# NVlabs/CenterPose

Measured on AMD Instinct MI355X. Metric: images/sec at 512x512 DLA-34 (backbone + heat-map decode + post-process + PnP), higher is better.
Workload: dtype f32 via split-f16 (f16x3) MFMA, f32 accumulate

## Files before the change

centerpose_amd/csrc/cp_common.h:

```cpp
#pragma once
#include <hip/hip_runtime.h>
#include <stdint.h>

#include "../../include/centerpose_hip_testing.h"

#if defined(__HIP_DEVICE_COMPILE__) && !defined(__gfx950__)
#error "centerpose_amd device code is written for gfx950 only (raw-buffer range-check semantics, MFMA shapes, LDS-DMA)"
#endif

#define CP_OK 0
#define CP_ERR_INVALID (-1)
#define CP_ERR_LAUNCH (-2)
#define CP_ERR_ALLOC (-3)
#define CP_ERR_STATE (-4)

enum CpAct : int {
    CP_ACT_NONE = 0,
    CP_ACT_RELU = 1,
    CP_ACT_SIGMOID = 2,
    CP_ACT_SIGMOID_FROM = 3,
};

enum CpStore : int {
    CP_STORE_NHWC = 0,
// ... 89 lines not shown
    int fuse_gbase[CP_MAX_HEAD_GROUP];
    int fuse_final;
    int fuse_gsig[CP_MAX_HEAD_GROUP];
    const float* fuse_gbias[CP_MAX_HEAD_GROUP];
    float* fuse_gout[CP_MAX_HEAD_GROUP];
    const unsigned* in_amax[CP_MAX_SRC];
    unsigned* out_amax;
    const float* fuse_w2_inv;
    int dbg;
    const float* offmask;
    const int* row_index;
    int rows_per_image, row_index_stride;
    const float* up_t;
    const float* up_wt;
    int up_ld, up_f;
};

int cp_launch_conv(const ConvParams& p, hipStream_t stream);
int cp_conv_tile_n(int cout);
int cp_conv_variant(const ConvParams& p);
int cp_launch_splitk_epilogue(const ConvParams& p, hipStream_t stream);
void cp_conv_geometry(const ConvParams& p, bool f16x3, int* tiles, int* nk);
const char* cp_conv_variant_name(int v);
#define CP_NUM_CONV_VARIANTS 46
#define CP_VARIANT_HEAD_ROWS 45
#define CP_VARIANT_DECONV_F32 43
#define CP_VARIANT_DECONV16 44
#define CP_VARIANT_STRM16 41
#define CP_VARIANT_LOWC1S 42
#define CP_VARIANT_GRU 26
bool cp_conv16_supported(const ConvParams& p);
int cp_launch_conv16(const ConvParams& p, hipStream_t stream);
int cp_conv16_variant(const ConvParams& p);
bool cp_halo16_supported(const ConvParams& p);
bool cp_halo16_fused_head_supported(const ConvParams& p);
int cp_launch_halo16_fused_head(const ConvParams& p, hipStream_t stream);
bool cp_halo16_gru_supported(const ConvParams& p);
int cp_launch_halo16_gru(const ConvParams& p, hipStream_t stream);
int cp_launch_halo16(const ConvParams& p, int bn, hipStream_t stream);
bool cp_strm16_supported(const ConvParams& p);
int cp_strm16_jobs(const ConvParams& p);
int cp_launch_strm16(const ConvParams& p, hipStream_t stream);
int cp_launch_dcn16(const ConvParams& p, int bn, hipStream_t stream);
bool cp_pw16_supported(const ConvParams& p);
int cp_launch_pw16(const ConvParams& p, hipStream_t stream);
bool cp_dcn16p_supported(const ConvParams& p);
int cp_dcn16p_blocks(const ConvParams& p);
int cp_launch_dcn16p(const ConvParams& p, hipStream_t stream);
bool cp_dcn16p_wide(const ConvParams& p);
#define CP_VARIANT_DCN16S 36
#define CP_VARIANT_M64N64 37
#define CP_VARIANT_DCN16PW 38
bool cp_dcn16s_supported(const ConvParams& p);
int cp_dcn16s_items(const ConvParams& p);
int cp_launch_dcn16s(const ConvParams& p, hipStream_t stream);
int cp_launch_frag16_repack(const void* w16, void* w16f, int CoutPad, int Kpad16, hipStream_t s);
#define CP_VARIANT_DCN16T 39
// ... 217 lines not shown
```

centerpose_amd/csrc/engine_forward.hip:

```cpp
#include "engine_model.h"

using namespace cp_engine;

namespace {

constexpr int kSplitTiles = 128, kSplitTarget = 384;
constexpr long kLeanMinPixels = 32768;

struct Fwd {
    cp_model* m;
    int B;
    hipStream_t s;
    double* gn_stats_out = nullptr;
    const float* gn_in_mr = nullptr;
    const float* gn_in_a = nullptr;
    const float* gn_in_d = nullptr;
    const float* gn_in_gamma = nullptr;
    const float* gn_in_beta = nullptr;
    int role = -1;
    const unsigned* gn_in_amax = nullptr;
    static constexpr int kMaxSlots = CP_AMAX_STRIDE;
    static constexpr size_t kSlotBytes = (size_t)CP_AMAX_SUB * CP_AMAX_STRIDE * sizeof(unsigned);
    Tensor slots_t;
    unsigned* slots = nullptr;
// ... 306 lines not shown
        const float* const some = (const float*)0x1000;
        ConvParams p = conv_params(B, H, W, &some, &C, 1, d.main, 1, 1, CP_ACT_RELU);
        if (p.Cin != d.main.CinP) return false;
        p.offmask = some;
        const unsigned* no_amax = nullptr;
        if (!conv_params_f16(p, d.main, &no_amax, true)) return false;
        p.store = CP_STORE_NHWC;
        p.ldo = d.main.Cout;
        p.up_t = p.up_wt = some;
        p.up_ld = t_c;
        p.up_f = f;
        p.splitk = plan_split(p, true, d.main);
        return p.splitk == 1 && cp_conv16_variant(p) == CP_VARIANT_DCN16T && cp_dcn16t_upadd_supported(p);
    }

    Tensor conv(const ConvW& w, const std::vector<const Tensor*>& srcs, int stride, int pad, int act,
                const Tensor* res = nullptr, const Tensor* offmask = nullptr, int act_from = 0,
                float* out_nchw = nullptr, int out_ld = 0, const UpFuse* up = nullptr) {
        const Tensor& x0 = *srcs[0];
        const int nsrc = (int)srcs.size();
        const float* src[CP_MAX_SRC];
        int src_c[CP_MAX_SRC];
        const unsigned* src_amax[CP_MAX_SRC];
        for (int i = 0; i < nsrc; ++i) {
            src[i] = srcs[i]->ptr();
            src_c[i] = srcs[i]->C;
            src_amax[i] = srcs[i]->amax;
        }
        ConvParams p = conv_params(B, x0.H, x0.W, src, src_c, nsrc, w, stride, pad, act);
        if (p.Cin != w.CinP) {
            chk(fail(CP_ERR_INVALID, "conv: channel mismatch"));
            return Tensor();
        }
// ... 35 lines not shown
            p.ldo = cstore;
            p.coff = 0;
        }
        Tensor partial;
        p.splitk = plan_split(p, use16, w);
        if (p.splitk > 1) {
            partial = make(p.splitk * p.CoutPad, p.Ho, p.Wo);
            p.partial = partial.ptr();
        }
        if (up) {
            p.up_t = up->t->ptr();
            p.up_wt = up->wt;
            p.up_ld = up->t->C;
            p.up_f = up->f;
        }
        auto launch = [&]() -> int {
            int rc = use16 ? cp_launch_conv16(p, s) : cp_launch_conv(p, s);
            if (rc == CP_OK && p.splitk > 1) rc = cp_launch_splitk_epilogue(p, s);
            return rc;
        };
        if (!m->dry)
            timed([&](cp_model::ProfRec& r) {
                r.variant = use16 ? cp_conv16_variant(p) : cp_conv_variant(p);
                r.role = role >= 0 ? role : offmask ? CP_ROLE_DCN : act == CP_ACT_SIGMOID_FROM ? CP_ROLE_DCN_OFFSET
                         : (w.KH == 1 && w.KW == 1) ? CP_ROLE_CONV1X1 : CP_ROLE_CONV;
                const double M = (double)B * p.Ho * p.Wo;
                const int cin_real = w.Cin;
                r.flops = 2.0 * M * w.Cout * (double)(w.KH * w.KW * cin_real);
                r.bytes = 4.0 * ((double)B * x0.H * x0.W * cin_real + M * w.Cout +
                                 (double)w.KH * w.KW * cin_real * w.Cout + (offmask ? M * 27 : 0.0) +
                                 (res ? M * w.Cout : 0.0) + (up ? (double)B * up->t->H * up->t->W * w.Cout : 0.0));
                r.M = (int)M; r.N = w.Cout; r.K = w.KH * w.KW * cin_real; r.kh = w.KH; r.stride = stride;
            }, launch);
        gn_stats_out = nullptr;
        gn_in_mr = nullptr;
        gn_in_a = nullptr;
        gn_in_d = nullptr;
        gn_in_amax = nullptr;
        role = -1;
        return out;
    }
    const ConvW& cw(const std::string& k) { return m->convs.at(k); }

    Tensor maxpool(const Tensor& x) {
        Tensor o = make(x.C, x.H / 2, x.W / 2);
        o.amax = x.amax;
        if (!m->dry) chk(cp_launch_maxpool2(x.ptr(), o.ptr(), B, x.H, x.W, x.C, s));
        return o;
    }

    Tensor basic_block(const std::string& p, const Tensor& x, int stride, const Tensor& residual) {
        Tensor t = conv(cw(p + ".conv1"), {&x}, stride, 1, CP_ACT_RELU);
        Tensor o = conv(cw(p + ".conv2"), {&t}, 1, 1, CP_ACT_RELU, &residual);
        tap(p, o);
        return o;
    }

    Tensor tree1(const std::string& p, const Tensor& x, int cin, int cout, int stride, bool level_root,
                 std::vector<const Tensor*> children, const Tensor* bottom_in = nullptr) {
        Tensor bottom_own;
        const Tensor* bottom = &x;
        if (stride > 1) {
            if (bottom_in) bottom = bottom_in;
            else {
                bottom_own = maxpool(x);
                bottom = &bottom_own;
            }
        }
        Tensor proj;
        const Tensor* residual = bottom;
        if (cin != cout) {
            proj = conv(cw(p + ".project"), {bottom}, 1, 0, CP_ACT_NONE);
            residual = &proj;
        }
        if (level_root) children.insert(children.begin(), bottom);
        Tensor x1 = basic_block(p + ".tree1", x, stride, *residual);
        proj = Tensor();
        Tensor x2 = basic_block(p + ".tree2", x1, 1, x1);
        std::vector<const Tensor*> srcs = {&x2, &x1};
        for (auto* c : children) srcs.push_back(c);
        Tensor o = conv(cw(p + ".root"), srcs, 1, 0, CP_ACT_RELU);
        tap(p + ".root", o);
        return o;
    }
    Tensor tree2(const std::string& p, const Tensor& x, int cin, int cout) {
        Tensor bottom = maxpool(x);
        Tensor x1 = tree1(p + ".tree1", x, cin, cout, 2, false, {}, &bottom);
        return tree1(p + ".tree2", x1, cout, cout, 1, false, {&bottom, &x1});
    }

    Tensor deform(const std::string& p, const Tensor& x, const UpFuse* up = nullptr) {
// ... 503 lines not shown
```

centerpose_amd/csrc/igemm.hip:

```cpp
#include "igemm_common.h"

namespace {

__device__ __forceinline__ float blend(float w1, float v1, float w2, float v2, float w3, float v3, float w4, float v4,
                                       float mk) {
    float s = __fadd_rn(__fadd_rn(__fadd_rn(__fmul_rn(w1, v1), __fmul_rn(w2, v2)), __fmul_rn(w3, v3)),
                        __fmul_rn(w4, v4));
    return __fmul_rn(s, mk);
}

template <int FRAG, int MT, int NT, int WM, int WN, bool DCN, bool ALIGNED, bool MULTISRC>
__global__ __launch_bounds__(NTHREADS, 3) void igemm_kernel(const ConvParams p, const int tiles_m, const int tiles_n) {
    typedef Frag<FRAG> F;
    typedef typename F::acc_t acc_t;
    constexpr int BM = FRAG * MT * WM, BN = FRAG * NT * WN;
    static_assert(WM * WN * 64 == NTHREADS, "4 waves");
    static_assert(!DCN || ALIGNED, "DCN needs aligned channels");
    static_assert(!MULTISRC || (ALIGNED && !DCN), "virtual concat only on the aligned plain-conv path");
    constexpr int LDA = BM + (FRAG == 16 ? 18 : 2);
    constexpr int LDB = BN + (FRAG == 16 ? 0 : 4);
    constexpr int A_SLOTS = BM * BK / 4 / NTHREADS;
    constexpr int B_F4 = BK * BN / 4;
    constexpr int B_SLOTS = (B_F4 + NTHREADS - 1) / NTHREADS;
    constexpr int A_SZ = BK * LDA, B_SZ = BK * LDB;
// ... 421 lines not shown
                      (!p.res || p.res_ld % 4 == 0) && p.splitk <= 32 && slab_bytes * 32 < (size_t)0xf0000000u &&
                      total / 4 < (size_t)0x7fffffff && !(p.dbg & CP_SEL_SPLITK_ELEMENTWISE);
    if (quad) {
        int g = (int)((total / 4 + 255) / 256);
        if (g > 4096) g = 4096;
        hipLaunchKernelGGL(splitk_epilogue4_kernel, dim3(g), dim3(256), 0, stream, p);
        return hipGetLastError() == hipSuccess ? CP_OK : CP_ERR_LAUNCH;
    }
    int g = (int)((total + 255) / 256);
    if (g > 4096) g = 4096;
    hipLaunchKernelGGL(splitk_epilogue_kernel, dim3(g), dim3(256), 0, stream, p);
    return hipGetLastError() == hipSuccess ? CP_OK : CP_ERR_LAUNCH;
}

int cp_launch_conv(const ConvParams& p, hipStream_t stream) {
    if (p.nsrc < 1 || p.nsrc > CP_MAX_SRC || p.Cin % 4 != 0 || p.up_t) return CP_ERR_INVALID;
    for (int s = 0; s < p.nsrc; ++s)
        if (p.src_c[s] % 4 != 0 || (p.nsrc > 1 && p.src_c[s] % BK != 0)) return CP_ERR_INVALID;
    const int bn = cp_conv_tile_n(p.Cout);
    if (p.offmask) {
        if (p.KH != 3 || p.KW != 3 || p.stride != 1 || p.pad != 1 || p.nsrc != 1 || p.Cin % BK != 0 ||
            p.H != p.Ho || p.W != p.Wo)
            return CP_ERR_INVALID;
        if (bn == 128) return launch<32, 2, 2, 2, 2, true>(p, stream);
        if (bn == 64) return launch<32, 2, 1, 2, 2, true>(p, stream);
        return CP_ERR_INVALID;
    }
    switch (bn) {
        case 16: return launch<16, 4, 1, 4, 1, false>(p, stream);
        case 32: return launch<32, 2, 1, 4, 1, false>(p, stream);
        case 64: return launch<32, 2, 1, 2, 2, false>(p, stream);
// ... 4 lines not shown
```

centerpose_amd/csrc/igemm16.hip:

```cpp
#include "igemm16_common.h"

namespace {

template <int MT, int NT, int WM, int WN, bool MULTISRC, bool FUSE = false, bool GNIN = false, bool GRU = false, bool ROWS = false>
__global__ __launch_bounds__(WM * WN * 64, 2) void igemm16p_kernel(const ConvParams p, const int tiles_m, const int tiles_n) {
    static_assert(!FUSE || (MT == 2 && NT == 2 && WM == 2 && WN == 2 && !MULTISRC), "fused head: 128x128 tiles");
    static_assert(!GRU || (MT == 1 && NT == 3 && WM == 4 && WN == 1 && !MULTISRC && !FUSE), "GRU: 128x96 tiles");
    static_assert(!ROWS || FUSE, "pixel lists: fused heads only");
    typedef Frag<32> F;
    typedef F::acc_t acc_t;
    constexpr int BM = 32 * MT * WM, BN = 32 * NT * WN;
    constexpr int NTH = WM * WN * 64;
    constexpr int RPP = NTH / 8;
    constexpr int A_SLOTS = BM * BK16 / 4 / NTH;
    constexpr int B_CHUNKS = BN * BK16 * 2 / 16;
    constexpr int B_SLOTS = (B_CHUNKS + NTH - 1) / NTH;
    constexpr bool B_PART = B_CHUNKS % NTH != 0;
    constexpr int A_SZ = BM * LDH, B_SZ = BN * LDH;
    constexpr int BUF = 2 * A_SZ + 2 * B_SZ;
    constexpr int NM = 3 * MT * NT;
    constexpr int NR = 2 * MT + 2 * NT;
    __shared__ __attribute__((aligned(16))) _Float16 lds[2 * BUF];

    const int tid = threadIdx.x;
// ... 539 lines not shown
    return (p.dbg & CP_SEL_DCN16S_ALWAYS) || cp_dcn16s_items(p) >= 4096;
}

static bool dcn16t_wanted(const ConvParams& p) {
    if ((p.dbg & CP_SEL_DCN16T_NEVER) || !dcn16p_wanted(p) || !cp_dcn16t_supported(p)) return false;
    if (p.dbg & CP_SEL_DCN16T_ALWAYS) return true;
    if (p.dbg & CP_SEL_DCN16S_ALWAYS) return false;
    return !cp_dcn16p_wide(p) && cp_dcn16p_blocks(p) >= 1024;
}

static bool strm16_wanted(const ConvParams& p) {
    if ((p.dbg & CP_SEL_STRM16_NEVER) || (p.dbg & CP_SEL_HALO_NEVER) || !cp_strm16_supported(p)) return false;
    return (p.dbg & CP_SEL_STRM16_ALWAYS) || cp_strm16_jobs(p) >= 1024;
}

static bool halo16_wanted(const ConvParams& p, int bn) {
    if ((p.dbg & CP_SEL_HALO_NEVER) || p.gn_in_a || !cp_halo16_supported(p)) return false;
    return bn == 32 || (p.w16f_hi && p.w16f_lo && !(p.dbg & CP_SEL_HALO_LDS_WEIGHTS)) || (p.dbg & CP_SEL_HALO_ALWAYS);
}

static bool pw16_wanted(const ConvParams& p) { return !(p.dbg & CP_SEL_PW16_NEVER) && cp_pw16_supported(p); }

bool cp_conv16_supported(const ConvParams& p) {
    if (!p.w16_hi || !p.w16_lo || p.Cin % BK16 != 0 || p.KH * p.KW > 32) return false;
    for (int s = 0; s < p.nsrc; ++s)
        if (p.src_c[s] % BK16 != 0) return false;
    const int bn = conv16_tile_n(p);
    if (bn < 32) return false;
    if (p.gn_in_mr) return false;
    if (p.gn_in_a || p.gn_in_d) {
        if (!p.gn_in_a || !p.gn_in_d || bn != 32 || p.KH != 1 || p.KW != 1 || p.pad != 0 || p.stride != 1 || p.nsrc != 1 ||
            p.offmask || (p.Ho * p.Wo) % 128 != 0)
            return false;
    }
    if (p.offmask && bn < 64) return false;
    for (int s = 0; s < p.nsrc; ++s)
        if ((size_t)p.B * p.H * p.W * p.src_c[s] * 4 >= (size_t)0xf0000000u) return false;
    if ((size_t)p.CoutPad * p.Kpad16 * 2 >= ((size_t)1 << 32)) return false;
    return true;
}

int cp_launch_conv16(const ConvParams& p, hipStream_t stream) {
    if (!cp_conv16_supported(p)) return CP_ERR_INVALID;
    if (p.up_t && !(p.offmask && dcn16t_wanted(p) && cp_dcn16t_upadd_supported(p))) return CP_ERR_INVALID;
    const int bn = conv16_tile_n(p);
    const bool cat = p.nsrc > 1;
    if (p.gn_in_a) {
        const int M = p.B * p.Ho * p.Wo;
        const int tiles_m = (M + 127) / 128, tiles_n = p.CoutPad / 32;
        hipLaunchKernelGGL((igemm16p_kernel<1, 1, 4, 1, false, false, true>),
                           dim3(tiles_m * tiles_n, p.splitk > 1 ? p.splitk : 1), dim3(NT16), 0, stream, p, tiles_m, tiles_n);
        return hipGetLastError() == hipSuccess ? CP_OK : CP_ERR_LAUNCH;
    }
    if (p.offmask) {
        if (p.KH != 3 || p.KW != 3 || p.stride != 1 || p.pad != 1 || p.nsrc != 1 || p.H != p.Ho || p.W != p.Wo)
            return CP_ERR_INVALID;
        if (dcn16t_wanted(p)) return cp_launch_dcn16t(p, stream);
        if (dcn16s_wanted(p)) return cp_launch_dcn16s(p, stream);
        if (dcn16p_wanted(p)) return cp_launch_dcn16p(p, stream);
// ... 112 lines not shown
```

centerpose_amd/csrc/ops.hip:

```cpp
#include "engine_model.h"

using namespace cp_engine;

namespace {

struct Carve {
    char* base;
    size_t off = 0;
    template <class T>
    T* take(size_t bytes) {
        T* p = base ? (T*)(base + off) : nullptr;
        off += align_up(bytes, 256);
        return p;
    }
};

constexpr size_t kSlotBytes = (size_t)CP_AMAX_SUB * CP_AMAX_STRIDE * sizeof(unsigned);

struct Pack16 {
    void *hi, *lo;
    float *wfwd, *winv, *sc16;
    unsigned* slot;
    void *fhi, *flo;
};
// ... 335 lines not shown
    d.wf = r.wf;
    d.hi = r.hi;
    d.lo = r.lo;
    d.scale = scale;
    d.scale16 = r.sc16;
    d.shift = shift;
    d.Cin = Cin;
    d.Cout = Cout;
    rc = cp_launch_deconv(deconv_launch(d, f16x3, x, f16x3 ? r.slot : nullptr, B, H, W, out, nullptr, act == CP_ACT_RELU), s);
    return rc == CP_OK ? CP_OK : fail(rc, "deconv launch failed (shape too large for 32-bit offsets?)");
}

int cp_conv2d_nhwc(cp_stream_t stream, const float* x, const float* w, const float* scale, const float* shift,
                   const float* residual, float* out, int B, int H, int W, int Cin, int Cout, int KH, int KW,
                   int stride, int pad, int act, void* workspace, size_t workspace_bytes) {
    if (!x || !w || !out || !workspace) return fail(CP_ERR_INVALID, "null argument");
    if (Cin % 4) return fail(CP_ERR_INVALID, "Cin must be a multiple of 4");
    Carve c{(char*)workspace};
    const Conv2dWs r = conv2d_carve(c, Cin, Cout, KH, KW);
    if (workspace_bytes < c.off) return fail(CP_ERR_INVALID, "workspace too small");
    hipStream_t s = (hipStream_t)stream;
    const int bn = cp_conv_tile_n(Cout);
    ConvW cw = conv_w_f32(r.wp, scale, shift, Cin, Cout, KH, KW);
    if ((scale || shift) && cw.CoutPad != Cout) return fail(CP_ERR_INVALID, "scale/shift need Cout % tile_n == 0");
    if (hipMemsetAsync(r.wp, 0, (size_t)cw.Kpad * cw.CoutPad * sizeof(float), s) != hipSuccess) return CP_ERR_LAUNCH;
    int rc = cp_launch_pack_weight(w, r.wp, Cout, Cin, KH * KW, Cin, cw.CoutPad, 0, s);
    if (rc != CP_OK) return rc;
    ConvParams p = conv_params(B, H, W, &x, &Cin, 1, cw, stride, pad, act);
    p.res = residual;
    p.res_ld = Cout;
    p.out = out;
    p.store = CP_STORE_NHWC;
    p.ldo = Cout;
    if (g_default_precision == CP_PREC_F16X3 && Cin % 32 == 0 && KH * KW <= 32 && bn >= 32) {
        rc = pack_f16x3(r.f16, w, scale, KH * KW, cw, x, (size_t)B * H * W * Cin, nullptr, 0, s);
        if (rc != CP_OK) return rc;
        const unsigned* slot = r.f16.slot;
        if (conv_params_f16(p, cw, &slot, true)) return cp_launch_conv16(p, s);
    }
    return cp_launch_conv(p, s);
}

size_t cp_conv2d_backward_workspace_bytes(int B, int H, int W, int Cin, int Cout, int KH, int KW, int stride, int pad,
                                          int need_grad_x) {
    if (const char* e = conv_bwd_shape_error(B, H, W, Cin, Cout, KH, KW, stride, pad)) {
        fail(CP_ERR_INVALID, e);
        return 0;
    }
    return cp_conv_backward_ws_bytes(B, H, W, Cin, Cout, KH, KW, stride, pad, need_grad_x);
}

int cp_conv2d_backward_nhwc(cp_stream_t stream, const float* x, const float* w, const float* y_or_null, const float* grad_out,
                            float* grad_x_or_null, float* grad_w, float* grad_bias_or_null, int B, int H, int W, int Cin,
                            int Cout, int KH, int KW, int stride, int pad, void* workspace, size_t workspace_bytes) {
// ... 133 lines not shown
```

centerpose_amd/hip.py:

```python
import contextlib
import ctypes
import enum
import os
from collections import OrderedDict
from collections.abc import Mapping

import torch

_HERE = os.path.dirname(os.path.abspath(__file__))
LIB_PATH = os.environ.get("CENTERPOSE_HIP_LIB") or os.path.join(_HERE, "libcenterpose_hip.so")

_lib = None
ABI_VERSION = 7

c_void_p = ctypes.c_void_p
c_int = ctypes.c_int
c_size_t = ctypes.c_size_t
c_char_p = ctypes.c_char_p


class TrackParams(ctypes.Structure):
    _fields_ = [(n, ctypes.c_double) for n in ("new_thresh", "pre_thresh", "R", "conf_lo", "conf_hi")] + \
               [(n, ctypes.c_int) for n in ("max_age", "kalman", "scale_pool", "use_pnp", "hps_uncertainty", "show_axes",
                                            "cat_rule", "render_hm_mode", "render_hmhp_mode", "pre_hm", "pre_hm_hp", "K",
# ... 76 lines not shown
         ctypes.POINTER(c_void_p))
    _sig(L.cp_model_set_param, c_int, c_void_p, c_char_p, c_void_p, ctypes.c_int64)
    _sig(L.cp_model_finalize, c_int, c_void_p)
    _sig(L.cp_model_destroy, None, c_void_p)
    _sig(L.cp_model_workspace_bytes, c_size_t, c_void_p, c_int, c_int, c_int)
    _sig(L.cp_model_forward, c_int, c_void_p, c_void_p, c_int, c_int, c_int, c_void_p, c_void_p, c_void_p, c_void_p,
         ctypes.POINTER(c_void_p), c_int, c_void_p, c_size_t)
    _sig(L.cp_model_forward_tap, c_int, c_void_p, c_void_p, c_int, c_int, c_int, c_void_p, c_void_p, c_void_p,
         c_void_p, ctypes.POINTER(c_void_p), c_int, c_void_p, c_size_t, c_char_p, c_void_p, ctypes.POINTER(c_int))
    _sig(L.cp_conv2d_workspace_bytes, c_size_t, c_int, c_int, c_int, c_int)
    _sig(L.cp_conv_transpose2d_workspace_bytes, c_size_t, c_int, c_int)
    _sig(L.cp_conv_transpose2d_nhwc, c_int, c_void_p, c_void_p, c_void_p, c_void_p, c_void_p, c_void_p,
         c_int, c_int, c_int, c_int, c_int, c_int, c_void_p, c_size_t)
    _sig(L.cp_conv2d_nhwc, c_int, c_void_p, c_void_p, c_void_p, c_void_p, c_void_p, c_void_p, c_void_p,
         *([c_int] * 10), c_void_p, c_size_t)
    _sig(L.cp_conv2d_backward_workspace_bytes, c_size_t, *([c_int] * 10))
    _sig(L.cp_conv2d_backward_nhwc, c_int, *([c_void_p] * 8), *([c_int] * 9), c_void_p, c_size_t)
    _sig(L.cp_batchnorm_workspace_bytes, c_size_t, *([c_int] * 4))
    _sig(L.cp_batchnorm_forward_nhwc, c_int, *([c_void_p] * 10), *([c_int] * 5), ctypes.c_float, ctypes.c_float, c_int, c_void_p,
         c_size_t)
    _sig(L.cp_batchnorm_backward_nhwc, c_int, *([c_void_p] * 11), *([c_int] * 5), c_void_p, c_size_t)
    _sig(L.cp_decode_workspace_bytes, c_size_t, c_int, c_int)
    _sig(L.cp_decode, c_int, c_void_p, c_int, c_int, c_int, *([c_void_p] * 11), c_int, c_int, c_int, ctypes.c_float,
         c_int, c_int, c_void_p, c_void_p, c_size_t)
    _sig(L.cp_decode_tiled_workspace_bytes, c_size_t, c_int, c_int, c_int, c_int)
    _sig(L.cp_decode_tiled, c_int, c_void_p, c_int, c_int, c_int, *([c_void_p] * 11), c_int, c_int, c_int, ctypes.c_float,
         c_int, c_int, c_void_p, c_void_p, c_size_t)
    _sig(L.cp_model_detect_workspace_bytes, c_size_t, c_void_p, c_int, c_int, c_int, c_int)
    _sig(L.cp_model_detect, c_int, c_void_p, c_void_p, c_int, c_int, c_int, c_void_p, c_void_p, c_void_p, c_void_p,
         ctypes.POINTER(c_void_p), c_int, c_int, c_int, ctypes.c_float, c_int, c_void_p, c_void_p, c_size_t, c_int)
# ... 69 lines not shown
            "cp_model_forward", "cp_model_forward_tap", "cp_conv2d_workspace_bytes", "cp_conv2d_nhwc",
            "cp_decode_workspace_bytes", "cp_decode", "cp_pnp_workspace_bytes", "cp_pnp_solve", "cp_model_profile", "cp_model_profile_read",
            "cp_kernel_variant_name", "cp_set_default_precision", "cp_model_set_precision", "cp_model_detect_workspace_bytes", "cp_model_detect", "cp_set_debug", "cp_preprocess", "cp_preprocess_batch", "cp_postprocess_workspace_bytes", "cp_postprocess", "cp_render_gaussians",
            "cp_model_profile_roles", "cp_role_name", "cp_pnp_from_post_workspace_bytes", "cp_pnp_from_post", "cp_resize_u8",
            "cp_abi_version", "cp_num_kernel_variants", "cp_num_roles", "cp_track_state_bytes", "cp_track_workspace_bytes",
            "cp_track_reset", "cp_track_step", "cp_track_status", "cp_linear_assignment", "cp_decode_tiled_workspace_bytes",
            "cp_decode_tiled", "cp_box_iou", "cp_box_eval", "cp_conv_transpose2d_workspace_bytes",
            "cp_conv_transpose2d_nhwc", "cp_dcnv2_backward_workspace_bytes", "cp_dcnv2_backward",
            "cp_pose_loss_workspace_bytes", "cp_pose_loss_forward", "cp_pose_loss_backward",
            "cp_pose_targets_workspace_bytes", "cp_pose_targets", "cp_model_lean_supported",
            "cp_model_detect_lean_workspace_bytes", "cp_model_detect_lean", "cp_model_dense_heads",
            "cp_model_heads_at_workspace_bytes", "cp_model_heads_at", "cp_decode_peaks_workspace_bytes", "cp_decode_peaks",
            "cp_decode_gathered", "cp_pose_heads_chunk_images", "cp_pose_heads_forward_workspace_bytes",
            "cp_pose_heads_forward", "cp_pose_heads_backward_workspace_bytes", "cp_pose_heads_backward",
            "cp_model_features", "cp_conv2d_backward_workspace_bytes", "cp_conv2d_backward_nhwc",
            "cp_batchnorm_workspace_bytes", "cp_batchnorm_forward_nhwc", "cp_batchnorm_backward_nhwc"]


def _check(rc, what):
    if rc != 0:
        msg = lib().cp_last_error().decode() if _lib is not None else ""
        raise RuntimeError("centerpose_hip: %s failed with code %d (%s)" % (what, rc, msg))


class KernelSel(enum.IntFlag):
    HEADS_SLABS = 0x00000001
    HEADS_WG_PER_HEAD = 0x00000002
    PW16_FRAG_A = 0x00000004
    SPLITK_ELEMENTWISE = 0x00000008
    TILE128_SMALL = 0x00000010
    NO_HEAD_FUSION = 0x00000020
# ... 165 lines not shown
    if need_feat_grad and grad_feat is None:
        grad_feat = torch.empty_like(feat, memory_format=torch.channels_last)
    if need_feat_grad and not (grad_feat.is_cuda and grad_feat.dtype == torch.float32 and grad_feat.shape == feat.shape and
                               grad_feat.is_contiguous(memory_format=torch.channels_last)):
        raise RuntimeError("pose_heads_backward: grad_feat must be a float32 channels_last tensor of feat's shape")
    nbytes = L.cp_pose_heads_backward_workspace_bytes(B, H, W, Cin, hid, n, cls_arr)
    if nbytes == 0:
        raise RuntimeError("pose_heads_backward: shape refused by the library (%s)" % L.cp_last_error().decode())
    ws = torch.empty(nbytes, dtype=torch.uint8, device=feat.device)
    rc = L.cp_pose_heads_backward(_stream(), _ptr(feat), n, *tables, cls_arr, goptr, *gtab,
                                  _ptr(grad_feat) if need_feat_grad else c_void_p(0), B, H, W, Cin, hid, _ptr(ws), nbytes)
    _check(rc, "cp_pose_heads_backward")
    return (grad_feat if need_feat_grad else None), grads


def conv2d_nhwc(x, w, scale=None, shift=None, residual=None, stride=1, pad=0, act=0):
    L = lib()
    x, w = _dev(x), _dev(w)
    B, H, W, Cin = x.shape
    Cout, _, KH, KW = w.shape
    Ho = (H + 2 * pad - KH) // stride + 1
    Wo = (W + 2 * pad - KW) // stride + 1
    out = torch.empty(B, Ho, Wo, Cout, device=x.device, dtype=torch.float32)
    nbytes = L.cp_conv2d_workspace_bytes(Cin, Cout, KH, KW)
    ws = torch.empty(nbytes, dtype=torch.uint8, device=x.device)
    scale = _dev(scale) if scale is not None else None
    shift = _dev(shift) if shift is not None else None
    residual = _dev(residual) if residual is not None else None
    rc = L.cp_conv2d_nhwc(_stream(), _ptr(x), _ptr(w), _ptr(scale), _ptr(shift), _ptr(residual), _ptr(out),
                          B, H, W, Cin, Cout, KH, KW, stride, pad, act, _ptr(ws), nbytes)
    _check(rc, "cp_conv2d_nhwc")
    return out


def conv2d_backward(x, w, grad_out, stride=1, pad=0, y=None, need_x_grad=True, need_bias_grad=True):
    L = lib()
    x, w, grad_out = _dev(x), _dev(w), _dev(grad_out)
    y = _dev(y) if y is not None else None
    if x.dim() != 4 or w.dim() != 4 or w.shape[1] != x.shape[3]:
        raise RuntimeError("conv2d_backward: x must be [B,H,W,Cin] and w [Cout,Cin,KH,KW], got %s and %s"
                           % (tuple(x.shape), tuple(w.shape)))
    B, H, W, Cin = x.shape
    Cout, _, KH, KW = w.shape
# ... 1082 lines not shown
```

include/centerpose_hip.h:

```cpp
#ifndef CENTERPOSE_HIP_H
#define CENTERPOSE_HIP_H

#include <stddef.h>
#include <stdint.h>

#ifdef __cplusplus
extern "C" {
#endif

typedef void* cp_stream_t;
typedef struct cp_model cp_model;

#define CP_OK 0
#define CP_ERR_INVALID (-1)
#define CP_ERR_LAUNCH (-2)
#define CP_ERR_ALLOC (-3)
#define CP_ERR_STATE (-4)

#define CP_ABI_VERSION 7
const char* cp_version(void);
int cp_abi_version(void);
const char* cp_last_error(void);

size_t cp_dcnv2_workspace_bytes(int B, int C, int H, int W, int Co);
// ... 77 lines not shown
#define CP_ROLE_HEAD 4
#define CP_ROLE_HEAD_FINAL 5
#define CP_ROLE_GRU 6
#define CP_ROLE_LOWC 7
#define CP_ROLE_DECODE 8
#define CP_ROLE_DECONV 9
#define CP_NUM_ROLES 10
int cp_num_roles(void);
int cp_model_profile_roles(cp_model* m, double* out, int num_roles);
const char* cp_role_name(int role);

size_t cp_conv2d_workspace_bytes(int Cin, int Cout, int KH, int KW);
int cp_conv2d_nhwc(cp_stream_t stream, const float* x, const float* w, const float* scale, const float* shift,
                   const float* residual, float* out, int B, int H, int W, int Cin, int Cout, int KH, int KW,
                   int stride, int pad, int act, void* workspace, size_t workspace_bytes);

size_t cp_conv2d_backward_workspace_bytes(int B, int H, int W, int Cin, int Cout, int KH, int KW, int stride, int pad,
                                          int need_grad_x);
int cp_conv2d_backward_nhwc(cp_stream_t stream, const float* x, const float* w, const float* y_or_null,
                            const float* grad_out, float* grad_x_or_null, float* grad_w, float* grad_bias_or_null, int B,
                            int H, int W, int Cin, int Cout, int KH, int KW, int stride, int pad, void* workspace,
                            size_t workspace_bytes);

size_t cp_batchnorm_workspace_bytes(int B, int H, int W, int C);
int cp_batchnorm_forward_nhwc(cp_stream_t stream, const float* x, const float* gamma_or_null, const float* beta_or_null,
                              const float* residual_or_null, float* running_mean_or_null, float* running_var_or_null,
                              float* y, float* save_mean, float* save_invstd, int B, int H, int W, int C, int training,
                              float momentum, float eps, int act, void* workspace, size_t workspace_bytes);
int cp_batchnorm_backward_nhwc(cp_stream_t stream, const float* x, const float* y_or_null, const float* grad_out,
                               const float* gamma_or_null, const float* save_mean, const float* save_invstd,
// ... 168 lines not shown
```

Measured before the change: 4539.

## Fuse 2x2 maxpool into streamed stride-2 3x3 conv kernel for tree entry

Adds a dedicated streamed stride-2 3x3 conv kernel (Cin 32 to Cout 64, split-f16 MFMA) that also writes the 2x2 max-pooled input as a side output. It is used at the DLA tree entry, where the stride-2 conv1 and the maxpool for the bottom path read the same input. This removes a separate maxpool launch and a second read of the large input tensor. The new kernel keeps weights in LDS, streams input rows through per-wave LDS buffers, and adds a selection heuristic and a new public API entry point. In exchange there is more special-case code, and it applies only to one narrow layer shape.

```diff
diff --git a/centerpose_amd/csrc/cp_common.h b/centerpose_amd/csrc/cp_common.h
--- a/centerpose_amd/csrc/cp_common.h
+++ b/centerpose_amd/csrc/cp_common.h
@@ -127,6 +127,7 @@
     const float* up_t;
     const float* up_wt;
     int up_ld, up_f;
+    float* pool_out;
 };
 
 int cp_launch_conv(const ConvParams& p, hipStream_t stream);
@@ -154,6 +155,10 @@
 bool cp_strm16_supported(const ConvParams& p);
 int cp_strm16_jobs(const ConvParams& p);
 int cp_launch_strm16(const ConvParams& p, hipStream_t stream);
+bool cp_igemm16s2_supported(const ConvParams& p);
+int cp_igemm16s2_jobs(const ConvParams& p);
+int cp_launch_igemm16s2(const ConvParams& p, hipStream_t stream);
+bool cp_conv16_pool_fusable(const ConvParams& p);
 int cp_launch_dcn16(const ConvParams& p, int bn, hipStream_t stream);
 bool cp_pw16_supported(const ConvParams& p);
 int cp_launch_pw16(const ConvParams& p, hipStream_t stream);
diff --git a/centerpose_amd/csrc/engine_forward.hip b/centerpose_amd/csrc/engine_forward.hip
--- a/centerpose_amd/csrc/engine_forward.hip
+++ b/centerpose_amd/csrc/engine_forward.hip
@@ -344,9 +344,22 @@
         return p.splitk == 1 && cp_conv16_variant(p) == CP_VARIANT_DCN16T && cp_dcn16t_upadd_supported(p);
     }
 
+    bool pool_fusable(const ConvW& w, int C, int H, int W) {
+        if (m->precision != CP_PREC_F16X3) return false;
+        const float* const some = (const float*)0x1000;
+        ConvParams p = conv_params(B, H, W, &some, &C, 1, w, 2, 1, CP_ACT_RELU);
+        if (p.Cin != w.CinP) return false;
+        const unsigned* no_amax = nullptr;
+        if (!conv_params_f16(p, w, &no_amax, true)) return false;
+        p.store = CP_STORE_NHWC;
+        p.ldo = w.Cout;
+        p.splitk = plan_split(p, true, w);
+        return p.splitk == 1 && cp_conv16_pool_fusable(p);
+    }
+
     Tensor conv(const ConvW& w, const std::vector<const Tensor*>& srcs, int stride, int pad, int act,
                 const Tensor* res = nullptr, const Tensor* offmask = nullptr, int act_from = 0,
-                float* out_nchw = nullptr, int out_ld = 0, const UpFuse* up = nullptr) {
+                float* out_nchw = nullptr, int out_ld = 0, const UpFuse* up = nullptr, const Tensor* pool = nullptr) {
         const Tensor& x0 = *srcs[0];
         const int nsrc = (int)srcs.size();
         const float* src[CP_MAX_SRC];
@@ -412,6 +425,7 @@
             p.up_ld = up->t->C;
             p.up_f = up->f;
         }
+        if (pool) p.pool_out = pool->ptr();
         auto launch = [&]() -> int {
             int rc = use16 ? cp_launch_conv16(p, s) : cp_launch_conv(p, s);
             if (rc == CP_OK && p.splitk > 1) rc = cp_launch_splitk_epilogue(p, s);
@@ -427,7 +441,8 @@
                 r.flops = 2.0 * M * w.Cout * (double)(w.KH * w.KW * cin_real);
                 r.bytes = 4.0 * ((double)B * x0.H * x0.W * cin_real + M * w.Cout +
                                  (double)w.KH * w.KW * cin_real * w.Cout + (offmask ? M * 27 : 0.0) +
-                                 (res ? M * w.Cout : 0.0) + (up ? (double)B * up->t->H * up->t->W * w.Cout : 0.0));
+                                 (res ? M * w.Cout : 0.0) + (up ? (double)B * up->t->H * up->t->W * w.Cout : 0.0) +
+                                 (pool ? M * cin_real : 0.0));
                 r.M = (int)M; r.N = w.Cout; r.K = w.KH * w.KW * cin_real; r.kh = w.KH; r.stride = stride;
             }, launch);
         gn_stats_out = nullptr;
@@ -449,6 +464,9 @@
 
     Tensor basic_block(const std::string& p, const Tensor& x, int stride, const Tensor& residual) {
         Tensor t = conv(cw(p + ".conv1"), {&x}, stride, 1, CP_ACT_RELU);
+        return basic_block_tail(p, t, residual);
+    }
+    Tensor basic_block_tail(const std::string& p, const Tensor& t, const Tensor& residual) {
         Tensor o = conv(cw(p + ".conv2"), {&t}, 1, 1, CP_ACT_RELU, &residual);
         tap(p, o);
         return o;
@@ -456,11 +474,16 @@
 
     Tensor tree1(const std::string& p, const Tensor& x, int cin, int cout, int stride, bool level_root,
                  std::vector<const Tensor*> children, const Tensor* bottom_in = nullptr) {
-        Tensor bottom_own;
+        Tensor bottom_own, entry;
         const Tensor* bottom = &x;
         if (stride > 1) {
             if (bottom_in) bottom = bottom_in;
-            else {
+            else if (stride == 2 && pool_fusable(cw(p + ".tree1.conv1"), x.C, x.H, x.W)) {
+                bottom_own = make(x.C, x.H / 2, x.W / 2);
+                bottom_own.amax = x.amax;
+                entry = conv(cw(p + ".tree1.conv1"), {&x}, 2, 1, CP_ACT_RELU, nullptr, nullptr, 0, nullptr, 0, nullptr, &bottom_own);
+                bottom = &bottom_own;
+            } else {
                 bottom_own = maxpool(x);
                 bottom = &bottom_own;
             }
@@ -472,7 +495,8 @@
             residual = &proj;
         }
         if (level_root) children.insert(children.begin(), bottom);
-        Tensor x1 = basic_block(p + ".tree1", x, stride, *residual);
+        Tensor x1 = entry.valid() ? basic_block_tail(p + ".tree1", entry, *residual) : basic_block(p + ".tree1", x, stride, *residual);
+        entry = Tensor();
         proj = Tensor();
         Tensor x2 = basic_block(p + ".tree2", x1, 1, x1);
         std::vector<const Tensor*> srcs = {&x2, &x1};
diff --git a/centerpose_amd/csrc/igemm.hip b/centerpose_amd/csrc/igemm.hip
--- a/centerpose_amd/csrc/igemm.hip
+++ b/centerpose_amd/csrc/igemm.hip
@@ -459,7 +459,7 @@
 }
 
 int cp_launch_conv(const ConvParams& p, hipStream_t stream) {
-    if (p.nsrc < 1 || p.nsrc > CP_MAX_SRC || p.Cin % 4 != 0 || p.up_t) return CP_ERR_INVALID;
+    if (p.nsrc < 1 || p.nsrc > CP_MAX_SRC || p.Cin % 4 != 0 || p.up_t || p.pool_out) return CP_ERR_INVALID;
     for (int s = 0; s < p.nsrc; ++s)
         if (p.src_c[s] % 4 != 0 || (p.nsrc > 1 && p.src_c[s] % BK != 0)) return CP_ERR_INVALID;
     const int bn = cp_conv_tile_n(p.Cout);
diff --git a/centerpose_amd/csrc/igemm16.hip b/centerpose_amd/csrc/igemm16.hip
--- a/centerpose_amd/csrc/igemm16.hip
+++ b/centerpose_amd/csrc/igemm16.hip
@@ -577,6 +577,11 @@
     return (p.dbg & CP_SEL_STRM16_ALWAYS) || cp_strm16_jobs(p) >= 1024;
 }
 
+bool cp_conv16_pool_fusable(const ConvParams& p) {
+    if ((p.dbg & CP_SEL_HALO_NEVER) || !cp_conv16_supported(p) || !cp_igemm16s2_supported(p)) return false;
+    return (p.dbg & CP_SEL_HALO_ALWAYS) || cp_igemm16s2_jobs(p) >= 1024;
+}
+
 static bool halo16_wanted(const ConvParams& p, int bn) {
     if ((p.dbg & CP_SEL_HALO_NEVER) || p.gn_in_a || !cp_halo16_supported(p)) return false;
     return bn == 32 || (p.w16f_hi && p.w16f_lo && !(p.dbg & CP_SEL_HALO_LDS_WEIGHTS)) || (p.dbg & CP_SEL_HALO_ALWAYS);
@@ -606,6 +611,8 @@
 int cp_launch_conv16(const ConvParams& p, hipStream_t stream) {
     if (!cp_conv16_supported(p)) return CP_ERR_INVALID;
     if (p.up_t && !(p.offmask && dcn16t_wanted(p) && cp_dcn16t_upadd_supported(p))) return CP_ERR_INVALID;
+    if (cp_conv16_pool_fusable(p)) return cp_launch_igemm16s2(p, stream);
+    if (p.pool_out) return CP_ERR_INVALID;
     const int bn = conv16_tile_n(p);
     const bool cat = p.nsrc > 1;
     if (p.gn_in_a) {
diff --git a/centerpose_amd/csrc/igemm16s2.hip b/centerpose_amd/csrc/igemm16s2.hip
--- /dev/null
+++ b/centerpose_amd/csrc/igemm16s2.hip
@@ -0,0 +1,258 @@
+#include "igemm16_common.h"
+
+namespace {
+
+constexpr int S2_W = 32;
+constexpr int S2_PITCH = 80;
+constexpr int S2_ODD = 34 * S2_PITCH;
+constexpr int S2_EVEN = 32 * S2_PITCH;
+constexpr int S2_ROWB = S2_ODD + S2_EVEN;
+constexpr int S2_G = 18;
+constexpr int S2_NF = 2;
+constexpr int S2_WB = 2 * S2_NF * S2_G * 1024;
+constexpr int S2_TAB = 128 * 4;
+constexpr int S2_WAVES = 8;
+constexpr int S2_LDS = S2_WB + S2_TAB + S2_WAVES * 2 * S2_ROWB;
+constexpr int S2_XP = 272;
+constexpr int S2_NLD = 9;
+static_assert(S2_LDS + 64 <= 160 * 1024, "one workgroup per CU");
+static_assert(32 * S2_XP <= 2 * S2_ROWB, "the output exchange lives in the wave's row buffer");
+
+__global__ __launch_bounds__(64 * S2_WAVES, 1) void igemm16s2_kernel(const ConvParams p, const int rows, const int strips,
+                                                                     const int bands, const int njobs) {
+    float* const pool_out = p.pool_out;
+    typedef Frag<32> F;
+    typedef F::acc_t acc_t;
+    extern __shared__ __attribute__((aligned(16))) unsigned char smem[];
+    const int tid = threadIdx.x, lane = tid & 63;
+    const int wid = __builtin_amdgcn_readfirstlane(tid >> 6);
+    float afwd, ainv;
+    conv_in_scale(p, &afwd, &ainv);
+    afwd = __uint_as_float(__builtin_amdgcn_readfirstlane(__float_as_uint(afwd)));
+    ainv = __uint_as_float(__builtin_amdgcn_readfirstlane(__float_as_uint(ainv)));
+    {
+        const u32x4* gh = reinterpret_cast<const u32x4*>(p.w16f_hi);
+        const u32x4* gl = reinterpret_cast<const u32x4*>(p.w16f_lo);
+        u32x4* ws = reinterpret_cast<u32x4*>(smem);
+        for (int i = tid; i < S2_NF * S2_G * 64; i += 64 * S2_WAVES) {
+            ws[i] = gh[i];
+            ws[S2_NF * S2_G * 64 + i] = gl[i];
+        }
+        float* tab = reinterpret_cast<float*>(smem + S2_WB);
+        if (tid < 64) {
+            tab[tid] = (p.scale ? p.scale[tid] : 1.f) * ainv;
+            tab[64 + tid] = p.shift ? p.shift[tid] : 0.f;
+        }
+    }
+    __syncthreads();
+    unsigned char* row_hi = smem + S2_WB + S2_TAB + wid * (2 * S2_ROWB);
+    unsigned char* row_lo = row_hi + S2_ROWB;
+    const unsigned char* w_hi = smem + lane * 16;
+    const unsigned char* w_lo = w_hi + S2_NF * S2_G * 1024;
+    const unsigned char* tab_b = smem + S2_WB;
+    const int px = lane & 31, kg = lane >> 5;
+    const int pr = lane >> 3, cq = lane & 7;
+    const unsigned img_b = (unsigned)p.H * (unsigned)p.W * 128u;
+    const float relu_floor = p.act == CP_ACT_RELU ? 0.f : -__builtin_inff();
+    const unsigned pool_b = pool_out ? (unsigned)p.Ho * (unsigned)p.Wo * 128u : 0u;
+    const int st_even = S2_ODD + pr * S2_PITCH + cq * 8, st_odd = (pr + 1) * S2_PITCH + cq * 8;
+    const int st_first = (pr == 0 ? 0 : 33) * S2_PITCH + cq * 8;
+    float amax = 0.f;
+
+    for (int job = wid * (int)gridDim.x + (int)blockIdx.x; job < njobs; job += (int)gridDim.x * S2_WAVES) {
+        int t = job;
+        const int sx = t % strips;
+        t /= strips;
+        const int band = t % bands, b = t / bands;
+        const int x0 = sx * S2_W, y0 = band * rows, y1 = min(y0 + rows, p.Ho);
+        const int j_first = 2 * y0 - 1, j_last = 2 * y1 - 1;
+        const __amdgpu_buffer_rsrc_t r_in = make_rsrc(p.src[0] + (size_t)b * p.H * p.W * 32, img_b);
+        const __amdgpu_buffer_rsrc_t r_out = make_rsrc(p.out + (size_t)b * p.Ho * p.Wo * p.ldo + p.coff, (unsigned)p.Ho * (unsigned)p.Wo * (unsigned)p.ldo * 4u);
+        const __amdgpu_buffer_rsrc_t r_pool = make_rsrc(pool_out ? pool_out + (size_t)b * p.Ho * p.Wo * 32 : p.out, pool_b);
+        unsigned cvo[S2_NLD];
+#pragma unroll
+        for (int k = 0; k < 4; ++k) {
+            const int c = 2 * (x0 + pr + 8 * k);
+            cvo[k] = c < p.W ? (unsigned)(c * 128 + cq * 16) : 0xffffffffu;
+            cvo[4 + k] = c < p.W ? (unsigned)((c + 1) * 128 + cq * 16) : 0xffffffffu;
+        }
+        cvo[8] = (pr == 0 && x0 > 0) ? (unsigned)((2 * x0 - 1) * 128 + cq * 16) : 0xffffffffu;
+        float4 pf[2][S2_NLD];
+        auto request = [&](int j, float4 (&v)[S2_NLD]) {
+            const bool row_ok = (j >= j_first) & (j <= j_last) & ((unsigned)j < (unsigned)p.H);
+            const int so = row_ok ? j * p.W * 128 : 0;
+#pragma unroll
+            for (int k = 0; k < S2_NLD; ++k) {
+                const u32x4 x = __builtin_amdgcn_raw_buffer_load_b128(r_in, (int)(row_ok ? cvo[k] : 0xffffffffu), so, 0);
+                v[k] = make_float4(__uint_as_float(x.x), __uint_as_float(x.y), __uint_as_float(x.z), __uint_as_float(x.w));
+            }
+        };
+        request(j_first - 1, pf[0]);
+        __builtin_amdgcn_sched_barrier(0);
+        request(j_first, pf[1]);
+        __builtin_amdgcn_sched_barrier(0);
+        acc_t acc0[S2_NF], acc1[S2_NF];
+#pragma unroll
+        for (int nf = 0; nf < S2_NF; ++nf)
+#pragma unroll
+            for (int r = 0; r < F::NACC; ++r) acc0[nf][r] = acc1[nf][r] = 0.f;
+        float4 hm[4];
+
+        auto stage = [&](const float4 (&buf)[S2_NLD]) {
+#pragma unroll
+            for (int k = 0; k < S2_NLD; ++k) {
+                const float4 v = buf[k];
+                const Split2 s0 = split2(v.x * afwd, v.y * afwd), s1 = split2(v.z * afwd, v.w * afwd);
+                const int o = k < 4 ? st_even + k * 8 * S2_PITCH : k < 8 ? st_odd + (k - 4) * 8 * S2_PITCH : st_first;
+                *reinterpret_cast<u32x2*>(row_hi + o) = u32x2{s0.hi, s1.hi};
+                *reinterpret_cast<u32x2*>(row_lo + o) = u32x2{s0.lo, s1.lo};
+            }
+        };
+        auto max4 = [](const float4& a, const float4& c) {
+            return make_float4(fmaxf(a.x, c.x), fmaxf(a.y, c.y), fmaxf(a.z, c.z), fmaxf(a.w, c.w));
+        };
+
+        for (int m = y0 - 1; m < y1; ++m) {
+            stage(pf[0]);
+#pragma unroll
+            for (int k = 0; k < 4; ++k) hm[k] = max4(pf[0][k], pf[0][4 + k]);
+            request(2 * m + 2, pf[0]);
+            __builtin_amdgcn_wave_barrier();
+#pragma unroll
+            for (int kw = 0; kw < 3; ++kw)
+#pragma unroll
+                for (int cg = 0; cg < 2; ++cg) {
+                    const int ao = (kw == 1 ? S2_ODD + px * S2_PITCH : (px + (kw >> 1)) * S2_PITCH) + cg * 32 + kg * 16;
+                    const h8 ah = *reinterpret_cast<const h8*>(row_hi + ao), al = *reinterpret_cast<const h8*>(row_lo + ao);
+                    h8 wh[S2_NF], wl[S2_NF];
+#pragma unroll
+                    for (int nf = 0; nf < S2_NF; ++nf) {
+                        const int g = nf * S2_G + (3 + kw) * 2 + cg;
+                        wh[nf] = *reinterpret_cast<const h8*>(w_hi + g * 1024);
+                        wl[nf] = *reinterpret_cast<const h8*>(w_lo + g * 1024);
+                    }
+#pragma unroll
+                    for (int nf = 0; nf < S2_NF; ++nf) acc0[nf] = __builtin_amdgcn_mfma_f32_32x32x16_f16(wh[nf], al, acc0[nf], 0, 0, 0);
+#pragma unroll
+                    for (int nf = 0; nf < S2_NF; ++nf) acc0[nf] = __builtin_amdgcn_mfma_f32_32x32x16_f16(wl[nf], ah, acc0[nf], 0, 0, 0);
+#pragma unroll
+                    for (int nf = 0; nf < S2_NF; ++nf) acc0[nf] = __builtin_amdgcn_mfma_f32_32x32x16_f16(wh[nf], ah, acc0[nf], 0, 0, 0);
+                }
+            __builtin_amdgcn_wave_barrier();
+            stage(pf[1]);
+            const unsigned okm = ~(unsigned)((m - y0) >> 31);
+            {
+                const unsigned prow = (unsigned)(m * p.Wo) * 128u, row_no = ~okm & 0x80000000u;
+#pragma unroll
+                for (int k = 0; k < 4; ++k) {
+                    const float4 v = max4(hm[k], max4(pf[1][k], pf[1][4 + k]));
+                    const int xo = x0 + pr + 8 * k;
+                    const unsigned col_no = xo < p.Wo ? 0u : 0x80000000u;
+                    const u32x4 pk = {__float_as_uint(v.x), __float_as_uint(v.y), __float_as_uint(v.z), __float_as_uint(v.w)};
+                    __builtin_amdgcn_raw_buffer_store_b128(pk, r_pool, (int)((prow + (unsigned)(xo * 128 + cq * 16)) | row_no | col_no), 0, 0);
+                }
+            }
+            request(2 * m + 3, pf[1]);
+            __builtin_amdgcn_wave_barrier();
+#pragma unroll
+            for (int kw = 0; kw < 3; ++kw)
+#pragma unroll
+                for (int cg = 0; cg < 2; ++cg) {
+                    const int ao = (kw == 1 ? S2_ODD + px * S2_PITCH : (px + (kw >> 1)) * S2_PITCH) + cg * 32 + kg * 16;
+                    const h8 ah = *reinterpret_cast<const h8*>(row_hi + ao), al = *reinterpret_cast<const h8*>(row_lo + ao);
+                    h8 wh[2][S2_NF], wl[2][S2_NF];
+#pragma unroll
+                    for (int nf = 0; nf < S2_NF; ++nf) {
+                        const int g2 = nf * S2_G + (6 + kw) * 2 + cg, g0 = nf * S2_G + kw * 2 + cg;
+                        wh[0][nf] = *reinterpret_cast<const h8*>(w_hi + g2 * 1024);
+                        wl[0][nf] = *reinterpret_cast<const h8*>(w_lo + g2 * 1024);
+                        wh[1][nf] = *reinterpret_cast<const h8*>(w_hi + g0 * 1024);
+                        wl[1][nf] = *reinterpret_cast<const h8*>(w_lo + g0 * 1024);
+                    }
+#pragma unroll
+                    for (int nf = 0; nf < S2_NF; ++nf) {
+                        acc0[nf] = __builtin_amdgcn_mfma_f32_32x32x16_f16(wh[0][nf], al, acc0[nf], 0, 0, 0);
+                        acc1[nf] = __builtin_amdgcn_mfma_f32_32x32x16_f16(wh[1][nf], al, acc1[nf], 0, 0, 0);
+                    }
+#pragma unroll
+                    for (int nf = 0; nf < S2_NF; ++nf) {
+                        acc0[nf] = __builtin_amdgcn_mfma_f32_32x32x16_f16(wl[0][nf], ah, acc0[nf], 0, 0, 0);
+                        acc1[nf] = __builtin_amdgcn_mfma_f32_32x32x16_f16(wl[1][nf], ah, acc1[nf], 0, 0, 0);
+                    }
+#pragma unroll
+                    for (int nf = 0; nf < S2_NF; ++nf) {
+                        acc0[nf] = __builtin_amdgcn_mfma_f32_32x32x16_f16(wh[0][nf], ah, acc0[nf], 0, 0, 0);
+                        acc1[nf] = __builtin_amdgcn_mfma_f32_32x32x16_f16(wh[1][nf], ah, acc1[nf], 0, 0, 0);
+                    }
+                }
+            __builtin_amdgcn_wave_barrier();
+            const float okf = __uint_as_float(okm & __float_as_uint(x0 + px < p.Wo ? 1.f : 0.f));
+#pragma unroll
+            for (int nf = 0; nf < S2_NF; ++nf)
+#pragma unroll
+                for (int g4 = 0; g4 < 4; ++g4) {
+                    const int n0 = 32 * nf + 8 * g4 + 4 * kg;
+                    const float4 sc = *reinterpret_cast<const float4*>(tab_b + n0 * 4), sh = *reinterpret_cast<const float4*>(tab_b + 256 + n0 * 4);
+                    float v[4] = {acc0[nf][4 * g4] * sc.x + sh.x, acc0[nf][4 * g4 + 1] * sc.y + sh.y,
+                                  acc0[nf][4 * g4 + 2] * sc.z + sh.z, acc0[nf][4 * g4 + 3] * sc.w + sh.w};
+#pragma unroll
+                    for (int e = 0; e < 4; ++e) {
+                        v[e] = fmaxf(v[e], relu_floor);
+                        amax = fmaxf(amax, fabsf(v[e]) * okf);
+                    }
+                    *reinterpret_cast<float4*>(row_hi + px * S2_XP + n0 * 4) = make_float4(v[0], v[1], v[2], v[3]);
+                }
+            __builtin_amdgcn_wave_barrier();
+            const unsigned row_out = (unsigned)(m * p.Wo * p.ldo) * 4u, row_no = ~okm & 0x80000000u;
+#pragma unroll
+            for (int i = 0; i < 8; ++i) {
+                const int pxo = (lane >> 4) + 4 * i;
+                const u32x4 pk = *reinterpret_cast<const u32x4*>(row_hi + pxo * S2_XP + (lane & 15) * 16);
+                const unsigned col_no = x0 + pxo < p.Wo ? 0u : 0x80000000u;
+                __builtin_amdgcn_raw_buffer_store_b128(pk, r_out, (int)((row_out + (unsigned)(((x0 + pxo) * p.ldo + (lane & 15) * 4) * 4)) | row_no | col_no), 0, 0);
+            }
+            __builtin_amdgcn_wave_barrier();
+#pragma unroll
+            for (int nf = 0; nf < S2_NF; ++nf) {
+                acc0[nf] = acc1[nf];
+#pragma unroll
+                for (int r = 0; r < F::NACC; ++r) acc1[nf][r] = 0.f;
+            }
+        }
+    }
+    if (p.out_amax) cp_amax_commit(p.out_amax, amax);
+}
+
+}
+
+bool cp_igemm16s2_supported(const ConvParams& p) {
+    return p.w16f_hi && p.w16f_lo && p.KH == 3 && p.KW == 3 && p.stride == 2 && p.pad == 1 && p.nsrc == 1 && p.Cin == 32 &&
+           p.src_c[0] == 32 && p.CoutPad == 64 && p.Cout == 64 && !p.offmask && !p.res && !p.gn_stats && !p.gn_in_a && !p.gn_in_mr &&
+           !p.gru_x3 && !p.fuse_w2_hi && !p.up_t && p.splitk <= 1 && p.tile_m != 64 && p.H % 2 == 0 && p.W % 2 == 0 && p.H >= 2 && p.W >= 2 &&
+           p.Ho == p.H / 2 && p.Wo == p.W / 2 && p.store == CP_STORE_NHWC && p.ldo % 4 == 0 && p.coff % 4 == 0 && p.coff + 64 <= p.ldo &&
+           p.Kpad16 == 288 && (p.act == CP_ACT_NONE || p.act == CP_ACT_RELU) &&
+           (size_t)p.H * p.W * 128 < (size_t)0x70000000u && (size_t)p.Ho * p.Wo * p.ldo * 4 < (size_t)0x70000000u;
+}
+
+int cp_igemm16s2_jobs(const ConvParams& p) { return p.B * ((p.Wo + S2_W - 1) / S2_W) * ((p.Ho + 15) / 16); }
+
+int cp_launch_igemm16s2(const ConvParams& p, hipStream_t stream) {
+    if (!cp_igemm16s2_supported(p)) return CP_ERR_INVALID;
+    static int cus_of[16] = {0};
+    int dev = 0;
+    if (hipGetDevice(&dev) != hipSuccess || dev < 0 || dev >= 16) return CP_ERR_LAUNCH;
+    if (!cus_of[dev]) {
+        hipDeviceProp_t prop;
+        if (hipFuncSetAttribute(reinterpret_cast<const void*>(&igemm16s2_kernel), hipFuncAttributeMaxDynamicSharedMemorySize, S2_LDS) != hipSuccess)
+            return CP_ERR_LAUNCH;
+        cus_of[dev] = (hipGetDeviceProperties(&prop, dev) == hipSuccess && prop.multiProcessorCount > 0) ? prop.multiProcessorCount : 256;
+    }
+    const int cus = cus_of[dev];
+    const int strips = (p.Wo + S2_W - 1) / S2_W;
+    const int rows = cp_igemm16s2_jobs(p) >= cus * S2_WAVES * 3 / 4 ? 16 : 8;
+    const int bands = (p.Ho + rows - 1) / rows;
+    const int njobs = p.B * strips * bands;
+    const int blocks = njobs < cus ? njobs : cus;
+    hipLaunchKernelGGL(igemm16s2_kernel, dim3(blocks), dim3(64 * S2_WAVES), S2_LDS, stream, p, rows, strips, bands, njobs);
+    return hipGetLastError() == hipSuccess ? CP_OK : CP_ERR_LAUNCH;
+}
diff --git a/centerpose_amd/csrc/ops.hip b/centerpose_amd/csrc/ops.hip
--- a/centerpose_amd/csrc/ops.hip
+++ b/centerpose_amd/csrc/ops.hip
@@ -373,6 +373,13 @@
 int cp_conv2d_nhwc(cp_stream_t stream, const float* x, const float* w, const float* scale, const float* shift,
                    const float* residual, float* out, int B, int H, int W, int Cin, int Cout, int KH, int KW,
                    int stride, int pad, int act, void* workspace, size_t workspace_bytes) {
+    return cp_conv2d_pool_nhwc(stream, x, w, scale, shift, residual, out, nullptr, B, H, W, Cin, Cout, KH, KW, stride, pad, act,
+                               workspace, workspace_bytes);
+}
+
+int cp_conv2d_pool_nhwc(cp_stream_t stream, const float* x, const float* w, const float* scale, const float* shift,
+                        const float* residual, float* out, float* pool_out, int B, int H, int W, int Cin, int Cout, int KH,
+                        int KW, int stride, int pad, int act, void* workspace, size_t workspace_bytes) {
     if (!x || !w || !out || !workspace) return fail(CP_ERR_INVALID, "null argument");
     if (Cin % 4) return fail(CP_ERR_INVALID, "Cin must be a multiple of 4");
     Carve c{(char*)workspace};
@@ -391,12 +398,18 @@
     p.out = out;
     p.store = CP_STORE_NHWC;
     p.ldo = Cout;
+    p.pool_out = pool_out;
+    const char* const no_pool = "pool_out: this launch does not run on the streamed stride-2 kernel (igemm16s2.hip)";
     if (g_default_precision == CP_PREC_F16X3 && Cin % 32 == 0 && KH * KW <= 32 && bn >= 32) {
         rc = pack_f16x3(r.f16, w, scale, KH * KW, cw, x, (size_t)B * H * W * Cin, nullptr, 0, s);
         if (rc != CP_OK) return rc;
         const unsigned* slot = r.f16.slot;
-        if (conv_params_f16(p, cw, &slot, true)) return cp_launch_conv16(p, s);
-    }
+        if (conv_params_f16(p, cw, &slot, true)) {
+            if (pool_out && !cp_conv16_pool_fusable(p)) return fail(CP_ERR_INVALID, no_pool);
+            return cp_launch_conv16(p, s);
+        }
+    }
+    if (pool_out) return fail(CP_ERR_INVALID, no_pool);
     return cp_launch_conv(p, s);
 }
 
diff --git a/centerpose_amd/hip.py b/centerpose_amd/hip.py
--- a/centerpose_amd/hip.py
+++ b/centerpose_amd/hip.py
@@ -114,6 +114,7 @@
          c_int, c_int, c_int, c_int, c_int, c_int, c_void_p, c_size_t)
     _sig(L.cp_conv2d_nhwc, c_int, c_void_p, c_void_p, c_void_p, c_void_p, c_void_p, c_void_p, c_void_p,
          *([c_int] * 10), c_void_p, c_size_t)
+    _sig(L.cp_conv2d_pool_nhwc, c_int, *([c_void_p] * 8), *([c_int] * 10), c_void_p, c_size_t)
     _sig(L.cp_conv2d_backward_workspace_bytes, c_size_t, *([c_int] * 10))
     _sig(L.cp_conv2d_backward_nhwc, c_int, *([c_void_p] * 8), *([c_int] * 9), c_void_p, c_size_t)
     _sig(L.cp_batchnorm_workspace_bytes, c_size_t, *([c_int] * 4))
@@ -213,7 +214,7 @@
             "cp_decode_gathered", "cp_pose_heads_chunk_images", "cp_pose_heads_forward_workspace_bytes",
             "cp_pose_heads_forward", "cp_pose_heads_backward_workspace_bytes", "cp_pose_heads_backward",
             "cp_model_features", "cp_conv2d_backward_workspace_bytes", "cp_conv2d_backward_nhwc",
-            "cp_batchnorm_workspace_bytes", "cp_batchnorm_forward_nhwc", "cp_batchnorm_backward_nhwc"]
+            "cp_batchnorm_workspace_bytes", "cp_batchnorm_forward_nhwc", "cp_batchnorm_backward_nhwc", "cp_conv2d_pool_nhwc"]
 
 
 def _check(rc, what):
@@ -409,7 +410,7 @@
     return (grad_feat if need_feat_grad else None), grads
 
 
-def conv2d_nhwc(x, w, scale=None, shift=None, residual=None, stride=1, pad=0, act=0):
+def conv2d_nhwc(x, w, scale=None, shift=None, residual=None, stride=1, pad=0, act=0, pool=False):
     L = lib()
     x, w = _dev(x), _dev(w)
     B, H, W, Cin = x.shape
@@ -422,6 +423,12 @@
     scale = _dev(scale) if scale is not None else None
     shift = _dev(shift) if shift is not None else None
     residual = _dev(residual) if residual is not None else None
+    if pool:
+        pooled = torch.empty(B, H // 2, W // 2, Cin, device=x.device, dtype=torch.float32)
+        rc = L.cp_conv2d_pool_nhwc(_stream(), _ptr(x), _ptr(w), _ptr(scale), _ptr(shift), _ptr(residual), _ptr(out),
+                                   _ptr(pooled), B, H, W, Cin, Cout, KH, KW, stride, pad, act, _ptr(ws), nbytes)
+        _check(rc, "cp_conv2d_pool_nhwc")
+        return out, pooled
     rc = L.cp_conv2d_nhwc(_stream(), _ptr(x), _ptr(w), _ptr(scale), _ptr(shift), _ptr(residual), _ptr(out),
                           B, H, W, Cin, Cout, KH, KW, stride, pad, act, _ptr(ws), nbytes)
     _check(rc, "cp_conv2d_nhwc")
diff --git a/include/centerpose_hip.h b/include/centerpose_hip.h
--- a/include/centerpose_hip.h
+++ b/include/centerpose_hip.h
@@ -115,6 +115,9 @@
 int cp_conv2d_nhwc(cp_stream_t stream, const float* x, const float* w, const float* scale, const float* shift,
                    const float* residual, float* out, int B, int H, int W, int Cin, int Cout, int KH, int KW,
                    int stride, int pad, int act, void* workspace, size_t workspace_bytes);
+int cp_conv2d_pool_nhwc(cp_stream_t stream, const float* x, const float* w, const float* scale, const float* shift,
+                        const float* residual, float* out, float* pool_out, int B, int H, int W, int Cin, int Cout, int KH,
+                        int KW, int stride, int pad, int act, void* workspace, size_t workspace_bytes);
 
 size_t cp_conv2d_backward_workspace_bytes(int B, int H, int W, int Cin, int Cout, int KH, int KW, int stride, int pad,
                                           int need_grad_x);
```

Result: no change. 4579 (median of 6 runs) (+0.9%).
